# DeepMed-Lab-ECNU/BCP

Measured on AMD Instinct MI355X. Metric: training volumes/sec (LA 112x112x80 V-Net, BCP self-training step), higher is better.
Workload: dtype f32 (fp16x2 split operands); 1 GPU; LA 3D V-Net BCP self-train step, per-GPU batch 4 (2 labeled), 112x112x80 patches, SGD m0.9 wd1e-4, EMA 0.99 (BASELINE.json configs[1]); global_batch=4, parallelism=dp1

## Files before the change

bcp_amd/_lib.py:

```python
from __future__ import annotations

import ctypes as C
import os

_HERE = os.path.dirname(os.path.abspath(__file__))
LIB_PATH = os.path.join(_HERE, "csrc", "libbcp_hip.so")

ABI_VERSION = 515

P = C.c_void_p
I = C.c_int
L = C.c_longlong
F = C.c_float
U64 = C.c_ulonglong
SZ = C.c_size_t

_SIGS = {
    "bcp_version": (I, []),
    "bcp_set_option": (I, [C.c_char_p, C.c_char_p]),
    "bcp_comm_available": (I, []),
    "bcp_comm_unique_id": (I, [P]),
    "bcp_comm_init_rank": (I, [C.POINTER(P), I, I, P]),
    "bcp_comm_count": (I, [P, C.POINTER(I)]),
    "bcp_allreduce_f32": (I, [P, P, C.c_longlong, P]),
# ... 50 lines not shown
    "bcp_conv3_fwd_stats": (I, [P, P, P, P, I, I, I, I, I, I, I, P, P, I, P, P]),
    "bcp_conv3_wgrad_workspace_bytes": (SZ, [I, I, I, I, I, I, I]),
    "bcp_conv3_wgrad": (I, [P, P, P, I, I, I, I, I, I, I, I, P, P, P, P]),
    "bcp_conv3_c1_fwd": (I, [P, P, P, P, I, I, I, I, I, P]),
    "bcp_conv3_c1_stat_rows": (I, [I, I, I, I, I, I]),
    "bcp_conv3_c1_fwd_stats": (I, [P, P, P, P, I, I, I, I, I, P, I, P]),
    "bcp_conv3_c1_norm_workspace_bytes": (SZ, [I, I, I, I, I, I]),
    "bcp_conv3_c1_norm_fwd": (I, [P, P, P, I, I, I, I, I, I, P, P, P, P, F, F, I, P, F, P, F, P, P, P, P, P]),
    "bcp_conv3_c1_norm_bwd": (I, [P, P, P, P, I, I, I, I, I, I, P, I, P, F, P, F, P, P, I, P, P, P]),
    "bcp_conv3_c1_norm_bwd_wgrad_workspace_bytes": (SZ, [I, I, I, I, I, I]),
    "bcp_conv3_c1_norm_bwd_wgrad": (I, [P, P, P, P, I, I, I, I, I, I, P, I, P, F, P, F, P, P, I, P, P, I, P]),
    "bcp_conv3_c1_wgrad": (I, [P, P, P, I, I, I, I, I, I, P, P]),
    "bcp_k2_pack_weight": (I, [P, P, I, I, I, P]),
    "bcp_k2_pack_desc": (I, [P, P, I, I, I, P]),
    "bcp_k2_pack_many": (I, [P, I, P]),
    "bcp_down_fwd": (I, [P, P, P, P, I, I, I, I, I, I, P]),
    "bcp_down_dgrad": (I, [P, P, P, I, I, I, I, I, I, I, P]),
    "bcp_up_fwd": (I, [P, P, P, P, I, I, I, I, I, I, P]),
    "bcp_up_dgrad": (I, [P, P, P, I, I, I, I, I, I, I, P]),
    "bcp_k2_stat_rows": (I, [I, I, I, I, I, I, I, I]),
    "bcp_down_fwd_stats": (I, [P, P, P, P, I, I, I, I, I, I, P, I, P]),
    "bcp_up_fwd_stats": (I, [P, P, P, P, I, I, I, I, I, I, P, I, P]),
    "bcp_k2_bwdstat_rows": (I, [I, I, I, I, I, I, I, I]),
    "bcp_down_dgrad_bwdstats": (I, [P, P, P, I, I, I, I, I, I, I, P, P, I, P, I, P]),
    "bcp_up_dgrad_bwdstats": (I, [P, P, P, I, I, I, I, I, I, I, P, P, I, P, I, P]),
    "bcp_up_norm_rows": (I, [I, I, I, I, I, I, I]),
    "bcp_up_norm_workspace_bytes": (SZ, [I, I, I, I, I, I, I]),
    "bcp_up_fwd_norm": (I, [P, P, P, I, I, I, I, I, I, I, P, P, P, P, F, F, I, P, P, P, P, P, P]),
    "bcp_up_norm_bwd": (I, [P, P, P, P, I, I, I, I, I, I, I, P, I, P, P, I, P, P, P]),
    "bcp_pw_fwd": (I, [P, P, P, P, L, I, I, P]),
# ... 91 lines not shown

class Binding:

    def __init__(self, path: str):
        if not os.path.exists(path):
            raise BcpError(
                f"{path} is missing: the HIP extension has not been built.  Run "
                "`python -c 'import __graft_entry__ as g; g.build()'` (hipcc --offload-arch=gfx950). "
                "There is no CPU fallback for the product path.")
        self.path = path
        self.cdll = C.CDLL(path)
        for name, (res, args) in _SIGS.items():
            fn = getattr(self.cdll, name)
            fn.restype = res
            fn.argtypes = args
        self._status_fns = {n for n, (r, _) in _SIGS.items() if r is I and n not in ("bcp_version", "bcp_conv3_stat_rows", "bcp_comm_available", "bcp_replay_count", "bcp_norm_slabs_ok", "bcp_conv3_planes", "bcp_conv3_fwd_nslabs", "bcp_conv3_bwdstat_rows", "bcp_conv3_c1_stat_rows", "bcp_k2_stat_rows", "bcp_k2_bwdstat_rows", "bcp_conv3_last_section", "bcp_up_norm_rows")}
        self._fns = {n: (getattr(self.cdll, n), n in self._status_fns) for n in _SIGS}
        got = int(self.cdll.bcp_version())
        if got != ABI_VERSION:
            raise BcpError(f"{path}: ABI revision {got}, this binding was written against {ABI_VERSION} (include/bcp_hip.h) -- rebuild: "
                           "python -c 'import __graft_entry__ as g; g.build()'")
        self._rec = None
        self.options_epoch = 0

    def last_error(self) -> str:
        return self.cdll.bcp_last_error().decode("utf-8", "replace")

    def set_option(self, name: str, value="") -> None:
        if isinstance(value, (tuple, list)):
            value = ",".join(str(int(v)) for v in value)
        self.call("bcp_set_option", name.encode(), str(value).encode())
# ... 26 lines not shown
```

bcp_amd/csrc/api.hip:

```cpp
#include "common.h"
#include "../../include/bcp_hip.h"
#include <cstring>

namespace bcp {
static thread_local char g_err[512] = "";
void set_error(const char* fmt, ...) {
  va_list ap;
  va_start(ap, fmt);
  vsnprintf(g_err, sizeof(g_err), fmt, ap);
  va_end(ap);
}
Options& options() {
  static Options o;
  return o;
}
}

extern "C" int bcp_version(void) { return BCP_ABI_VERSION; }

extern "C" int bcp_set_option(const char* name, const char* value) {
  BCP_REQUIRE(name && value, "bcp_set_option: null argument");
  bcp::Options& o = bcp::options();
  const bcp::Options def;
  long long v[5] = {0, 0, 0, 0, 0};
  const int n = sscanf(value, "%lld,%lld,%lld,%lld,%lld", &v[0], &v[1], &v[2], &v[3], &v[4]);
  const bool reset = n <= 0;
#define BCP_OPT_INT(field) if (!strcmp(name, #field)) { o.field = reset ? def.field : (int)v[0]; return BCP_OK; }
  BCP_OPT_INT(conv3_p) BCP_OPT_INT(splitk) BCP_OPT_INT(conv3_b6_flat_sk) BCP_OPT_INT(conv3_b6_cfg2d) BCP_OPT_INT(conv3_b6_w22) BCP_OPT_INT(conv3_b6_pipe) BCP_OPT_INT(conv3_b6_cin16max) BCP_OPT_INT(res_pcu) BCP_OPT_INT(res_nt) BCP_OPT_INT(wgrad_nt)
  BCP_OPT_INT(tn_groups) BCP_OPT_INT(cc_tile) BCP_OPT_INT(pack_sections) BCP_OPT_INT(cc_select_blocks) BCP_OPT_INT(conv3_b6) BCP_OPT_INT(conv3_b6_levels) BCP_OPT_INT(conv3_b6_direct) BCP_OPT_INT(conv3_b6_flat) BCP_OPT_INT(conv3_b6_minvox) BCP_OPT_INT(wgrad_b6) BCP_OPT_INT(wgrad_b6_minvox) BCP_OPT_INT(wgrad_b6_levels) BCP_OPT_INT(wgrad_b6_slots) BCP_OPT_INT(cc_border_dedupe) BCP_OPT_INT(cc_count_tile) BCP_OPT_INT(cc_fuse_select) BCP_OPT_INT(gemm_walk) BCP_OPT_INT(gemm_pipe) BCP_OPT_INT(gemm_stat_r) BCP_OPT_INT(norm_apply_cap) BCP_OPT_INT(norm_apply_vec) BCP_OPT_INT(k2_stats) BCP_OPT_INT(k2_bwd_stats) BCP_OPT_INT(up_recompute) BCP_OPT_INT(wgrad_b6_deep) BCP_OPT_INT(wgrad_b6_deep_nt) BCP_OPT_INT(wgrad_b6_deep_slots) BCP_OPT_INT(wgrad_b6_deep_tile) BCP_OPT_INT(norm_slabs) BCP_OPT_INT(conv3_f16) BCP_OPT_INT(fuse_bwd_stats) BCP_OPT_INT(conv3_xcd) BCP_OPT_INT(mix_c1) BCP_OPT_INT(whatif) BCP_OPT_INT(c3d16_form) BCP_OPT_INT(norm_own) BCP_OPT_INT(wgrad_reduce_flat) BCP_OPT_INT(norm_fin_rows) BCP_OPT_INT(norm_fuse_fin)
#undef BCP_OPT_INT
  if (!strcmp(name, "conv3_sk_elems")) { o.conv3_sk_elems = reset ? def.conv3_sk_elems : v[0]; return BCP_OK; }
  if (!strcmp(name, "res_tile2d_vox")) { o.res_tile2d_vox = reset ? def.res_tile2d_vox : v[0]; return BCP_OK; }
  if (!strcmp(name, "conv3_cfg")) {
    BCP_REQUIRE(reset || n == 4, "bcp_set_option: conv3_cfg wants TD,TH,TW,NT");
    for (int i = 0; i < 4; ++i) o.conv3_cfg[i] = reset ? 0 : (int)v[i];
    return BCP_OK;
  }
  if (!strcmp(name, "wgrad_tile")) {
    BCP_REQUIRE(reset || n >= 3, "bcp_set_option: wgrad_tile wants TD,TH,TW[,min_voxels,max_voxels]");
    for (int i = 0; i < 5; ++i) o.wgrad_tile[i] = def.wgrad_tile[i];
    for (int i = 0; i < n && !reset; ++i) o.wgrad_tile[i] = v[i];
    return BCP_OK;
  }
  bcp::set_error("bcp_set_option: unknown option '%s'", name);
// ... 74 lines not shown
```

bcp_amd/csrc/common.h:

```cpp
#pragma once
#include <hip/hip_runtime.h>
#include <cstdarg>
#include <cstdint>
#include <cstdio>

#define BCP_OK 0
#define BCP_EINVAL (-1)
#define BCP_ELAUNCH (-2)
#define BCP_EUNSUP (-3)

typedef float f32x4 __attribute__((ext_vector_type(4)));

namespace bcp {

void set_error(const char* fmt, ...);

#define BCP_REQUIRE(cond, ...)          \
  do {                                  \
    if (!(cond)) {                      \
      ::bcp::set_error(__VA_ARGS__);    \
      return BCP_EINVAL;                \
    }                                   \
  } while (0)

// ... 46 lines not shown
  int up_recompute = 0;
  int k2_bwd_stats = 0;
  int norm_fuse_fin = 1;
  int norm_fin_rows = 128;
  int gemm_pipe = 1;
  int gemm_stat_r = 0;
  int gemm_walk = 0;
  int cc_border_dedupe = 1;
  int cc_count_tile = 0;
  int cc_fuse_select = 1;
  int norm_apply_cap = 2048;
  int norm_apply_vec = 4;
  int wgrad_reduce_flat = 1;
  int norm_own = 0;
  int c3d16_form = 1;
  int whatif = 0;
  int wgrad_b6_levels = 15;
};
Options& options();

__device__ __forceinline__ unsigned char plabel_bin_of(float x0, float x1, float thres) {
  const float m = fmaxf(x0, x1);
  const float e0 = expf(x0 - m), e1 = expf(x1 - m);
  const float p1 = e1 / (e0 + e1);
  return (p1 >= thres) ? 1 : 0;
}
__device__ __forceinline__ unsigned char plabel_argmax4_of(float x0, float x1, float x2, float x3) {
  const float m = fmaxf(fmaxf(x0, x1), fmaxf(x2, x3));
  const float e0 = expf(x0 - m), e1 = expf(x1 - m), e2 = expf(x2 - m), e3 = expf(x3 - m);
  const float s = e0 + e1 + e2 + e3;
// ... 8 lines not shown


static inline int cdiv(long long a, long long b) { return (int)((a + b - 1) / b); }
static inline bool aligned16(const void* p) { return (reinterpret_cast<uintptr_t>(p) & 15u) == 0; }

#ifndef BCP_LDS_BARRIER
#define BCP_LDS_BARRIER() asm volatile("s_waitcnt lgkmcnt(0)\n\ts_barrier" ::: "memory")
#endif

#ifndef BCP_GLDS16
typedef __attribute__((address_space(3))) void* bcp_lds_ptr_t;
#define BCP_GLDS16(gsrc, lds_wave_base) __builtin_amdgcn_global_load_lds((gsrc), (bcp_lds_ptr_t)(lds_wave_base), 16, 0, 0)
#define BCP_VM_LDS_BARRIER(N) asm volatile("s_waitcnt vmcnt(%0) lgkmcnt(0)\n\ts_barrier" ::"n"(N) : "memory")
#endif

#ifndef BCP_S_SLEEP
#define BCP_S_SLEEP(n) __builtin_amdgcn_s_sleep(n)
#endif

__device__ __forceinline__ float wave_sum(float v) {
#pragma unroll
  for (int o = 32; o > 0; o >>= 1) v += __shfl_xor(v, o);
  return v;
}
__device__ __forceinline__ double wave_sum(double v) {
#pragma unroll
  for (int o = 32; o > 0; o >>= 1) v += __shfl_xor(v, o);
  return v;
}

// ... 78 lines not shown
```

bcp_amd/csrc/gemm.hip:

```cpp
#include "common.h"
#include <cstring>
#include <cstdlib>
#include "../../include/bcp_hip.h"

namespace bcp {

enum { MAP_PLAIN = 0, MAP_PATCH = 1 };

struct RowMap {
  float* p;
  int mode;
  int L;
  int Cs;
  int D, H, W;
  __device__ __forceinline__ long long base(int m) const {
    if (mode == MAP_PLAIN) return (long long)m * L;
    const int Wc = W >> 1, Hc = H >> 1, Dc = D >> 1;
    const int wc = m % Wc, hc = (m / Wc) % Hc, dc = (m / (Wc * Hc)) % Dc, n = m / (Wc * Hc * Dc);
    return ((((long long)n * D + 2 * dc) * H + 2 * hc) * W + 2 * wc) * Cs;
  }
  __device__ __forceinline__ long long off16(int q16) const {
    if (mode == MAP_PLAIN) return q16;
    const int s = q16 / Cs, c = q16 - s * Cs;
    const int pw = s & 1, ph = (s >> 1) & 1, pd = s >> 2;
// ... 130 lines not shown
    for (int nt = 0; nt < NT; ++nt) {
      float* o = crow + C.off16(n0 + nt * 16);
      float4 v = make_float4(acc[nt][0], acc[nt][1], acc[nt][2], acc[nt][3]);
      if (bias) {
        const float4 bv = ld4(bias + (n0 + nt * 16) % bias_mod + lg * 4);
        v.x += bv.x; v.y += bv.y; v.z += bv.z; v.w += bv.w;
      }
      if (accumulate) { const float4 p = ld4(o); v.x += p.x; v.y += p.y; v.z += p.z; v.w += p.w; }
      if constexpr (STATS <= 2 || STATS == 7) st4(o, v);
      if constexpr (STATS == 3) {
        p1[nt][0] += v.x; p2[nt][0] = fmaf(v.x, v.x, p2[nt][0]);
        p1[nt][1] += v.y; p2[nt][1] = fmaf(v.y, v.y, p2[nt][1]);
        p1[nt][2] += v.z; p2[nt][2] = fmaf(v.z, v.z, p2[nt][2]);
        p1[nt][3] += v.w; p2[nt][3] = fmaf(v.w, v.w, p2[nt][3]);
      }
      if constexpr (STATS >= 4) {
        const int cb = (n0 + nt * 16) % st.C + lg * 4;
        const long long pi = (long long)(blockIdx.x / st.wpg) * st.C + cb, GC = (long long)st.G * st.C;
        const float4 mu = ld4(st.bstats + pi), rs = ld4(st.bstats + GC + pi), sc = ld4(st.bstats + 2 * GC + pi), sh = ld4(st.bstats + 3 * GC + pi);
        const float yy[4] = {v.x, v.y, v.z, v.w};
        const float m4[4] = {mu.x, mu.y, mu.z, mu.w}, r4[4] = {rs.x, rs.y, rs.z, rs.w}, s4[4] = {sc.x, sc.y, sc.z, sc.w}, h4[4] = {sh.x, sh.y, sh.z, sh.w};
        float ov[4];
        if constexpr (STATS == 4) {
          float4 rv = make_float4(0.f, 0.f, 0.f, 0.f);
          if (st.aux) rv = ld4(st.aux + (o - C.p));
          const float rr[4] = {rv.x, rv.y, rv.z, rv.w};
#pragma unroll
          for (int r = 0; r < 4; ++r) {
            const float z = (yy[r] - m4[r]) * s4[r] + h4[r];
            ov[r] = act_fwd(z, st.act);
            if (st.aux) ov[r] += rr[r];
// ... 85 lines not shown
    const int g = blockIdx.x / st.wpg, row = (blockIdx.x % st.wpg) * st.ysets + blockIdx.y / ychan;
    const int c0 = (blockIdx.y % ychan) * CT;
    if ((int)threadIdx.x < ntc * 16) {
      const int c = threadIdx.x;
      double a = 0.0, b = 0.0;
#pragma unroll
      for (int w = 0; w < 4; ++w) { a += Ss[(w * CT + c) * 2]; b += Ss[(w * CT + c) * 2 + 1]; }
      double* dst = st.partial + (((long long)g * st.nb + row) * st.C + c0 + c) * 2;
      dst[0] = a;
      dst[1] = b;
    }
    }
  }
}

template <int NT>
__global__ __launch_bounds__(256) void k_gemm_tn(RowMap A, RowMap B, float* __restrict__ partial, int M, int K, int N,
                                                 int rows_per_group) {
  constexpr int CT = NT * 16;
  constexpr int AS2 = 64 + 16;
  constexpr int BS2 = (CT % 32 == 0) ? CT + 16 : CT;
  constexpr int NB4 = (64 * (CT / 4) + 255) / 256;
  __shared__ __attribute__((aligned(16))) float As[64 * AS2];
  __shared__ __attribute__((aligned(16))) float Bs[64 * BS2];
  __shared__ long long rbase[2][2][64];
  const int lane = threadIdx.x & 63, wave = threadIdx.x >> 6;
  const int li = lane & 15, lg = lane >> 4;
  const int grp = blockIdx.x, k0 = blockIdx.y * 64, n0 = blockIdx.z * CT;
  const int r_begin = grp * rows_per_group;
  int r_end = r_begin + rows_per_group;
// ... 457 lines not shown
  if (i < C) out[i] = (accumulate ? out[i] : 0.f) + (float)accum[i];
}

static RowMap make_map(const float* p, int mode, int L, int Cs, int D, int H, int W) {
  RowMap m;
  m.p = const_cast<float*>(p);
  m.mode = mode; m.L = L; m.Cs = Cs; m.D = D; m.H = H; m.W = W;
  return m;
}

static int pick_nt(int N, long long row_blocks) {
  int nt = 4;
  while (nt > 1 && (N % (nt * 16) != 0)) nt >>= 1;
  while (nt > 1 && row_blocks * (N / (nt * 16)) < 256) nt >>= 1;
  return nt;
}

static int launch_nn(RowMap A, const float* Bp, const float* bias, RowMap C, int M, int K, int N, int bias_mod, int accumulate,
                     hipStream_t s) {
  const int rb = cdiv(M, 64);
  const int nt = pick_nt(N, rb);
  const dim3 grid(rb, N / (nt * 16));
  const GemmStats none{nullptr, 0, 0, 0, 0, 0, nullptr, nullptr, 0, 0, nullptr, nullptr, nullptr, 0};
  const int walk = options().gemm_walk;
  if (walk > 0 && (long long)rb * grid.y >= 2LL * walk) {
    int R = cdiv((long long)rb * grid.y, walk);
    if (R > 16) R = 16;
    GemmStats st = none;
    st.R = R;
    st.pipe = options().gemm_pipe;
    const dim3 g2(cdiv(rb, R), grid.y);
    if (nt == 4) hipLaunchKernelGGL((k_gemm_nn<4, 7>), g2, dim3(256), 0, s, A, Bp, bias, C, M, K, N, bias_mod, accumulate, st);
    else if (nt == 2) hipLaunchKernelGGL((k_gemm_nn<2, 7>), g2, dim3(256), 0, s, A, Bp, bias, C, M, K, N, bias_mod, accumulate, st);
    else hipLaunchKernelGGL((k_gemm_nn<1, 7>), g2, dim3(256), 0, s, A, Bp, bias, C, M, K, N, bias_mod, accumulate, st);
    return 0;
  }
  if (nt == 4) hipLaunchKernelGGL((k_gemm_nn<4>), grid, dim3(256), 0, s, A, Bp, bias, C, M, K, N, bias_mod, accumulate, none);
  else if (nt == 2) hipLaunchKernelGGL((k_gemm_nn<2>), grid, dim3(256), 0, s, A, Bp, bias, C, M, K, N, bias_mod, accumulate, none);
  else hipLaunchKernelGGL((k_gemm_nn<1>), grid, dim3(256), 0, s, A, Bp, bias, C, M, K, N, bias_mod, accumulate, none);
  return 0;
}

struct StatPlan { int nt, R, wpg, ysets, nb; };
static bool stat_plan(StatPlan& p, int M, int N, int Cout, int groups) {
  if (groups < 1 || M % groups) return false;
  const int mpg = M / groups;
  if (mpg % 64) return false;
  const int bpg = mpg / 64;
  p.nt = pick_nt(N, (long long)bpg * groups);
  const int CT = p.nt * 16;
  if (Cout % 16 || (Cout < CT && CT % Cout) || (Cout > CT && Cout % CT) || N % Cout) return false;
// ... 98 lines not shown
  BCP_REQUIRE(w && bp && desc_out && Cin > 0 && Cout > 0, "bcp_k2_pack_desc: bad argument");
  BCP_REQUIRE(Cin % 16 == 0 && Cout % 16 == 0, "bcp_k2_pack_desc: channels must be multiples of 16");
  static_assert(sizeof(GemmPackDesc) == 64, "descriptor layout is part of the ABI");
  GemmPackDesc d;
  d.w = w; d.bp = bp;
  BCP_REQUIRE(k2_pack_geometry(Cin, Cout, kind, d.K, d.N, d.ix) == 0, "bcp_k2_pack_desc: unknown kind %d", kind);
  memcpy(desc_out, &d, sizeof(d));
  return BCP_OK;
}

extern "C" int bcp_k2_pack_many(const void* descs_dev, int n, void* stream) {
  BCP_REQUIRE(descs_dev && n > 0, "bcp_k2_pack_many: bad argument");
  hipLaunchKernelGGL(k_pack_gemm_b_many, dim3(256, n), dim3(256), 0, (hipStream_t)stream, (const GemmPackDesc*)descs_dev);
  BCP_CHECK_LAUNCH("bcp_k2_pack_many");
  return BCP_OK;
}

extern "C" int bcp_down_fwd(const float* x, const float* bp, const float* bias, float* y, int N, int D, int H, int W, int Cin,
                            int Cout, void* stream) {
  BCP_REQUIRE(x && bp && y, "bcp_down_fwd: null pointer");
  BCP_REQUIRE(D % 2 == 0 && H % 2 == 0 && W % 2 == 0 && Cin % 16 == 0 && Cout % 16 == 0, "bcp_down_fwd: bad shape");
  const int M = N * (D / 2) * (H / 2) * (W / 2);
  launch_nn(make_map(x, MAP_PATCH, 8 * Cin, Cin, D, H, W), bp, bias, make_map(y, MAP_PLAIN, Cout, 0, 0, 0, 0), M, 8 * Cin, Cout,
            Cout, 0, (hipStream_t)stream);
  BCP_CHECK_LAUNCH("bcp_down_fwd");
  return BCP_OK;
}

extern "C" int bcp_k2_stat_rows(int kind, int N, int D, int H, int W, int Cin, int Cout, int groups) {
  if (N < 1 || D < 2 || H < 2 || W < 2 || (D | H | W) & 1 || Cin % 16 || Cout % 16 || Cin < 16 || Cout < 16 || groups < 1) return 0;
// ... 341 lines not shown
```

bcp_amd/csrc/replay_shapes.inc:

```
BCP_SHAPE(pifpppiiiiiipp, (void*, int, float, void*, void*, void*, int, int, int, int, int, int, void*, void*), (a[0].p, a[1].i, a[2].f, a[3].p, a[4].p, a[5].p, a[6].i, a[7].i, a[8].i, a[9].i, a[10].i, a[11].i, a[12].p, a[13].p))
BCP_SHAPE(piiiipiip, (void*, int, int, int, int, void*, int, int, void*), (a[0].p, a[1].i, a[2].i, a[3].i, a[4].i, a[5].p, a[6].i, a[7].i, a[8].p))
BCP_SHAPE(piiiippp, (void*, int, int, int, int, void*, void*, void*), (a[0].p, a[1].i, a[2].i, a[3].i, a[4].i, a[5].p, a[6].p, a[7].p))
BCP_SHAPE(piiippp, (void*, int, int, int, void*, void*, void*), (a[0].p, a[1].i, a[2].i, a[3].i, a[4].p, a[5].p, a[6].p))
BCP_SHAPE(piliippfipppppippp, (void*, int, long long, int, int, void*, void*, float, int, void*, void*, void*, void*, void*, int, void*, void*, void*), (a[0].p, a[1].i, a[2].l, a[3].i, a[4].i, a[5].p, a[6].p, a[7].f, a[8].i, a[9].p, a[10].p, a[11].p, a[12].p, a[13].p, a[14].i, a[15].p, a[16].p, a[17].p))
BCP_SHAPE(pilippppffiplpfpfppppiplpp, (void*, int, long long, int, void*, void*, void*, void*, float, float, int, void*, long long, void*, float, void*, float, void*, void*, void*, void*, int, void*, long long, void*, void*), (a[0].p, a[1].i, a[2].l, a[3].i, a[4].p, a[5].p, a[6].p, a[7].p, a[8].f, a[9].f, a[10].i, a[11].p, a[12].l, a[13].p, a[14].f, a[15].p, a[16].f, a[17].p, a[18].p, a[19].p, a[20].p, a[21].i, a[22].p, a[23].l, a[24].p, a[25].p))
BCP_SHAPE(pilippppffiplpipppippp, (void*, int, long long, int, void*, void*, void*, void*, float, float, int, void*, long long, void*, int, void*, void*, void*, int, void*, void*, void*), (a[0].p, a[1].i, a[2].l, a[3].i, a[4].p, a[5].p, a[6].p, a[7].p, a[8].f, a[9].f, a[10].i, a[11].p, a[12].l, a[13].p, a[14].i, a[15].p, a[16].p, a[17].p, a[18].i, a[19].p, a[20].p, a[21].p))
BCP_SHAPE(pilppilippppffiplpfpfpppppp, (void*, int, long long, void*, void*, int, long long, int, void*, void*, void*, void*, float, float, int, void*, long long, void*, float, void*, float, void*, void*, void*, void*, void*, void*), (a[0].p, a[1].i, a[2].l, a[3].p, a[4].p, a[5].i, a[6].l, a[7].i, a[8].p, a[9].p, a[10].p, a[11].p, a[12].f, a[13].f, a[14].i, a[15].p, a[16].l, a[17].p, a[18].f, a[19].p, a[20].f, a[21].p, a[22].p, a[23].p, a[24].p, a[25].p, a[26].p))
BCP_SHAPE(pip, (void*, int, void*), (a[0].p, a[1].i, a[2].p))
BCP_SHAPE(pipiiiippp, (void*, int, void*, int, int, int, int, void*, void*, void*), (a[0].p, a[1].i, a[2].p, a[3].i, a[4].i, a[5].i, a[6].i, a[7].p, a[8].p, a[9].p))
BCP_SHAPE(pipp, (void*, int, void*, void*), (a[0].p, a[1].i, a[2].p, a[3].p))
BCP_SHAPE(pippiiiiipip, (void*, int, void*, void*, int, int, int, int, int, void*, int, void*), (a[0].p, a[1].i, a[2].p, a[3].p, a[4].i, a[5].i, a[6].i, a[7].i, a[8].i, a[9].p, a[10].i, a[11].p))
BCP_SHAPE(plffipp, (void*, long long, float, float, int, void*, void*), (a[0].p, a[1].l, a[2].f, a[3].f, a[4].i, a[5].p, a[6].p))
BCP_SHAPE(plffiup, (void*, long long, float, float, int, unsigned long long, void*), (a[0].p, a[1].l, a[2].f, a[3].f, a[4].i, a[5].u, a[6].p))
BCP_SHAPE(plipipp, (void*, long long, int, void*, int, void*, void*), (a[0].p, a[1].l, a[2].i, a[3].p, a[4].i, a[5].p, a[6].p))
BCP_SHAPE(plippppfipipp, (void*, long long, int, void*, void*, void*, void*, float, int, void*, int, void*, void*), (a[0].p, a[1].l, a[2].i, a[3].p, a[4].p, a[5].p, a[6].p, a[7].f, a[8].i, a[9].p, a[10].i, a[11].p, a[12].p))
BCP_SHAPE(plippppfippp, (void*, long long, int, void*, void*, void*, void*, float, int, void*, void*, void*), (a[0].p, a[1].l, a[2].i, a[3].p, a[4].p, a[5].p, a[6].p, a[7].f, a[8].i, a[9].p, a[10].p, a[11].p))
BCP_SHAPE(plllppipiiiiippfpp, (void*, long long, long long, long long, void*, void*, int, void*, int, int, int, int, int, void*, void*, float, void*, void*), (a[0].p, a[1].l, a[2].l, a[3].l, a[4].p, a[5].p, a[6].i, a[7].p, a[8].i, a[9].i, a[10].i, a[11].i, a[12].i, a[13].p, a[14].p, a[15].f, a[16].p, a[17].p))
BCP_SHAPE(plllppipiiiiipppp, (void*, long long, long long, long long, void*, void*, int, void*, int, int, int, int, int, void*, void*, void*, void*), (a[0].p, a[1].l, a[2].l, a[3].l, a[4].p, a[5].p, a[6].i, a[7].p, a[8].i, a[9].i, a[10].i, a[11].i, a[12].i, a[13].p, a[14].p, a[15].p, a[16].p))
BCP_SHAPE(pp, (void*, void*), (a[0].p, a[1].p))
BCP_SHAPE(ppiiiiiiiiiiiiiiip, (void*, void*, int, int, int, int, int, int, int, int, int, int, int, int, int, int, int, void*), (a[0].p, a[1].p, a[2].i, a[3].i, a[4].i, a[5].i, a[6].i, a[7].i, a[8].i, a[9].i, a[10].i, a[11].i, a[12].i, a[13].i, a[14].i, a[15].i, a[16].i, a[17].p))
BCP_SHAPE(ppiiiiiip, (void*, void*, int, int, int, int, int, int, void*), (a[0].p, a[1].p, a[2].i, a[3].i, a[4].i, a[5].i, a[6].i, a[7].i, a[8].p))
BCP_SHAPE(ppiiiiiipiip, (void*, void*, int, int, int, int, int, int, void*, int, int, void*), (a[0].p, a[1].p, a[2].i, a[3].i, a[4].i, a[5].i, a[6].i, a[7].i, a[8].p, a[9].i, a[10].i, a[11].p))
BCP_SHAPE(ppiiiiiipp, (void*, void*, int, int, int, int, int, int, void*, void*), (a[0].p, a[1].p, a[2].i, a[3].i, a[4].i, a[5].i, a[6].i, a[7].i, a[8].p, a[9].p))
BCP_SHAPE(ppiiiiip, (void*, void*, int, int, int, int, int, void*), (a[0].p, a[1].p, a[2].i, a[3].i, a[4].i, a[5].i, a[6].i, a[7].p))
// ... 47 lines not shown
```

bcp_amd/hip_ops.py:

```python
from __future__ import annotations

import ctypes as C
import os

import torch

from . import _lib

ACT_NONE, ACT_RELU, ACT_LRELU = 0, 1, 2
LOSS_LA, LOSS_ACDC = 0, 1
PACK_DOWN_FWD, PACK_DOWN_DGRAD, PACK_UP_FWD, PACK_UP_DGRAD, PACK_PW_FWD, PACK_PW_DGRAD = range(6)
WG_DOWN, WG_UP, WG_PW = range(3)
CAST_I64_U8, CAST_F32_U8, CAST_U8_F32, CAST_U8_I64 = range(4)


AMAX_FLOATS, AMAX_STRIDE = 1024, 32
EDT_NOSITE = 1 << 30


def amax_slots(value, device):
    a = torch.zeros(AMAX_FLOATS, dtype=torch.float32, device=device)
    a[0] = value
    return a

# ... 693 lines not shown
    def k2_pack(self, w, Cin, Cout, kind):
        self._chk(w)
        bp = torch.empty(w.numel(), dtype=torch.float32, device=w.device)
        self.b.call("bcp_k2_pack_weight", _p(w), _p(bp), Cin, Cout, kind, self.stream(w))
        return bp

    def k2_pack_desc(self, w, bp, Cin, Cout, kind):
        import ctypes
        buf = ctypes.create_string_buffer(64)
        self.b.call("bcp_k2_pack_desc", _p(w), _p(bp), Cin, Cout, kind, ctypes.addressof(buf))
        return buf.raw

    def k2_pack_many(self, descs, n):
        self._chk(descs)
        self.b.call("bcp_k2_pack_many", _p(descs), int(n), self.stream(descs))

    def down_fwd(self, x, bp, bias, Cout, out=None):
        self._chk(x, bp, bias)
        N, D, H, W, Cin = x.shape
        if out is None:
            out = torch.empty((N, D // 2, H // 2, W // 2, Cout), dtype=torch.float32, device=x.device)
        self.b.call("bcp_down_fwd", _p(x), _p(bp), _p(bias), _p(out), N, D, H, W, Cin, Cout, self.stream(x))
        return self._no_amax(out)

    def k2_stat_rows(self, kind, xshape, Cout, groups):
        N, D, H, W, Cin = xshape
        fine = (D, H, W) if kind == 0 else (2 * D, 2 * H, 2 * W)
        return self._ws_bytes("bcp_k2_stat_rows", int(kind), N, fine[0], fine[1], fine[2], Cin, Cout, int(groups))

    def k2_fwd_stats(self, kind, x, bp, bias, Cout, groups):
# ... 365 lines not shown
```

include/bcp_hip.h:

```cpp
#ifndef BCP_HIP_H
#define BCP_HIP_H
#include <stddef.h>
#include <stdint.h>

#ifdef __cplusplus
extern "C" {
#endif

#define BCP_OK 0
#define BCP_EINVAL (-1)
#define BCP_ELAUNCH (-2)
#define BCP_EUNSUP (-3)

enum { BCP_ACT_NONE = 0, BCP_ACT_RELU = 1, BCP_ACT_LRELU = 2 };
enum { BCP_LOSS_LA = 0, BCP_LOSS_ACDC = 1 };
enum { BCP_CAST_I64_U8 = 0, BCP_CAST_F32_U8 = 1, BCP_CAST_U8_F32 = 2, BCP_CAST_U8_I64 = 3 };
enum { BCP_PACK_DOWN_FWD = 0, BCP_PACK_DOWN_DGRAD = 1, BCP_PACK_UP_FWD = 2, BCP_PACK_UP_DGRAD = 3, BCP_PACK_PW_FWD = 4, BCP_PACK_PW_DGRAD = 5 };
enum { BCP_WG_DOWN = 0, BCP_WG_UP = 1, BCP_WG_PW = 2 };

#define BCP_ABI_VERSION 515
int bcp_version(void);
const char* bcp_last_error(void);
int bcp_set_option(const char* name, const char* value);
int bcp_device_arch(char* buf, int n);
int bcp_event_create(void** ev);
int bcp_event_record(void* ev, void* stream);
int bcp_event_elapsed_ms(void* start, void* stop, float* ms);
int bcp_event_destroy(void* ev);

int bcp_mix_box(const float* a, const float* b, float* out, int N, int D, int H, int W, int C, const int* box6 , void* stream);

int bcp_mask_boxes(uint8_t* out, int N, int D, int H, int W, const int* boxes , int K, int complement, void* stream);
int bcp_mix_mask(const float* a, const float* b, const uint8_t* mask, float* out, int N, int D, int H, int W, long long mask_sample_stride,
                 void* stream);

// ... 109 lines not shown
int bcp_conv3_c1_norm_bwd(const float* x, const float* w, const float* bias_or_null, const float* da, int N, int D, int H, int W, int KD,
                          int groups, const float* stats, int act, const uint8_t* elem_mask, float elem_scale,
                          const unsigned long long* mask_seed_or_null, float mask_p_keep, float* dgamma, float* dbeta,
                          int accumulate, void* workspace, float* dy, void* stream);
int bcp_conv3_c1_wgrad(const float* x, const float* dy, float* dw, int N, int D, int H, int W, int KD, int accumulate, void* workspace,
                       void* stream);
size_t bcp_conv3_c1_norm_bwd_wgrad_workspace_bytes(int N, int D, int H, int W, int KD, int groups);
int bcp_conv3_c1_norm_bwd_wgrad(const float* x, const float* w, const float* bias_or_null, const float* da, int N, int D, int H, int W, int KD,
                                int groups, const float* stats, int act, const uint8_t* elem_mask, float elem_scale,
                                const unsigned long long* mask_seed_or_null, float mask_p_keep, float* dgamma, float* dbeta,
                                int accumulate, void* workspace, float* dw, int dw_accumulate, void* stream);

int bcp_k2_pack_weight(const float* w, float* bp , int Cin, int Cout, int kind, void* stream);
int bcp_k2_pack_desc(const float* w, float* bp, int Cin, int Cout, int kind, void* desc_out );
int bcp_k2_pack_many(const void* descs_dev, int n, void* stream);
int bcp_down_fwd(const float* x, const float* bp, const float* bias, float* y, int N, int D, int H, int W, int Cin, int Cout, void* stream);
int bcp_down_dgrad(const float* dy, const float* bp, float* dx, int N, int D, int H, int W, int Cin, int Cout, int accumulate, void* stream);
int bcp_up_fwd(const float* x, const float* bp, const float* bias, float* y, int N, int D, int H, int W, int Cin, int Cout, void* stream);
int bcp_k2_stat_rows(int kind, int N, int D, int H, int W, int Cin, int Cout, int groups);
int bcp_down_fwd_stats(const float* x, const float* bp, const float* bias, float* y, int N, int D, int H, int W, int Cin, int Cout, double* stat_partial, int groups, void* stream);
int bcp_up_fwd_stats(const float* x, const float* bp, const float* bias, float* y, int N, int D, int H, int W, int Cin, int Cout, double* stat_partial, int groups, void* stream);
int bcp_k2_bwdstat_rows(int kind, int N, int D, int H, int W, int Cin, int Cout, int groups);
int bcp_down_dgrad_bwdstats(const float* dy, const float* bp, float* dx, int N, int D, int H, int W, int Cin, int Cout, int accumulate, const float* y_prev, const float* stats_prev, int act, double* stat_partial, int groups, void* stream);
int bcp_up_dgrad_bwdstats(const float* dy, const float* bp, float* dx, int N, int D, int H, int W, int Cin, int Cout, int accumulate, const float* y_prev, const float* stats_prev, int act, double* stat_partial, int groups, void* stream);
int bcp_up_norm_rows(int N, int D, int H, int W, int Cin, int Cout, int groups);
size_t bcp_up_norm_workspace_bytes(int N, int D, int H, int W, int Cin, int Cout, int groups);
int bcp_up_fwd_norm(const float* x, const float* bp, const float* bias, int N, int D, int H, int W, int Cin, int Cout, int groups, const float* gamma, const float* beta, float* running_mean, float* running_var, float momentum, float eps, int act, const float* residual_or_null, float* stats, void* workspace, float* out, float* amax_out_or_null, void* stream);
int bcp_up_norm_bwd(const float* x, const float* bp, const float* bias, const float* da, int N, int D, int H, int W, int Cin, int Cout, int groups, const float* stats, int act, float* dgamma, float* dbeta, int accumulate, void* workspace, float* dy, void* stream);
int bcp_up_dgrad(const float* dy, const float* bp, float* dx, int N, int D, int H, int W, int Cin, int Cout, int accumulate, void* stream);
int bcp_pw_fwd(const float* x, const float* bp, const float* bias_or_null, float* y, long long rows, int Cin, int Cout, void* stream);
// ... 83 lines not shown
```

Measured before the change: 814.1 volumes/s.

## Add multi-stage async LDS-pipelined NN GEMM kernel for large-K down/up convs

Adds a new NN GEMM kernel that prefetches four K-stages of A and B into LDS through direct global-to-LDS loads, with graded vmcnt barriers and explicit ds_read_b128 register staging ahead of the MFMA chain. It is enabled by default (gemm_kpipe=1) for non-stats, non-walk NN launches with K of at least 256, and aims to hide global memory latency in the k2 down/up/pointwise GEMMs. The kernel uses far more LDS, which may limit occupancy to two workgroups per CU. A path-query entry point and an option are also added.

```diff
diff --git a/bcp_amd/_lib.py b/bcp_amd/_lib.py
--- a/bcp_amd/_lib.py
+++ b/bcp_amd/_lib.py
@@ -6,7 +6,7 @@
 _HERE = os.path.dirname(os.path.abspath(__file__))
 LIB_PATH = os.path.join(_HERE, "csrc", "libbcp_hip.so")
 
-ABI_VERSION = 515
+ABI_VERSION = 516
 
 P = C.c_void_p
 I = C.c_int
@@ -88,6 +88,7 @@
     "bcp_k2_pack_weight": (I, [P, P, I, I, I, P]),
     "bcp_k2_pack_desc": (I, [P, P, I, I, I, P]),
     "bcp_k2_pack_many": (I, [P, I, P]),
+    "bcp_gemm_nn_path": (I, [L, I, I]),
     "bcp_down_fwd": (I, [P, P, P, P, I, I, I, I, I, I, P]),
     "bcp_down_dgrad": (I, [P, P, P, I, I, I, I, I, I, I, P]),
     "bcp_up_fwd": (I, [P, P, P, P, I, I, I, I, I, I, P]),
@@ -209,7 +210,7 @@
             fn = getattr(self.cdll, name)
             fn.restype = res
             fn.argtypes = args
-        self._status_fns = {n for n, (r, _) in _SIGS.items() if r is I and n not in ("bcp_version", "bcp_conv3_stat_rows", "bcp_comm_available", "bcp_replay_count", "bcp_norm_slabs_ok", "bcp_conv3_planes", "bcp_conv3_fwd_nslabs", "bcp_conv3_bwdstat_rows", "bcp_conv3_c1_stat_rows", "bcp_k2_stat_rows", "bcp_k2_bwdstat_rows", "bcp_conv3_last_section", "bcp_up_norm_rows")}
+        self._status_fns = {n for n, (r, _) in _SIGS.items() if r is I and n not in ("bcp_version", "bcp_conv3_stat_rows", "bcp_comm_available", "bcp_replay_count", "bcp_norm_slabs_ok", "bcp_conv3_planes", "bcp_conv3_fwd_nslabs", "bcp_conv3_bwdstat_rows", "bcp_conv3_c1_stat_rows", "bcp_k2_stat_rows", "bcp_k2_bwdstat_rows", "bcp_conv3_last_section", "bcp_up_norm_rows", "bcp_gemm_nn_path")}
         self._fns = {n: (getattr(self.cdll, n), n in self._status_fns) for n in _SIGS}
         got = int(self.cdll.bcp_version())
         if got != ABI_VERSION:
diff --git a/bcp_amd/csrc/api.hip b/bcp_amd/csrc/api.hip
--- a/bcp_amd/csrc/api.hip
+++ b/bcp_amd/csrc/api.hip
@@ -27,7 +27,7 @@
   const bool reset = n <= 0;
 #define BCP_OPT_INT(field) if (!strcmp(name, #field)) { o.field = reset ? def.field : (int)v[0]; return BCP_OK; }
   BCP_OPT_INT(conv3_p) BCP_OPT_INT(splitk) BCP_OPT_INT(conv3_b6_flat_sk) BCP_OPT_INT(conv3_b6_cfg2d) BCP_OPT_INT(conv3_b6_w22) BCP_OPT_INT(conv3_b6_pipe) BCP_OPT_INT(conv3_b6_cin16max) BCP_OPT_INT(res_pcu) BCP_OPT_INT(res_nt) BCP_OPT_INT(wgrad_nt)
-  BCP_OPT_INT(tn_groups) BCP_OPT_INT(cc_tile) BCP_OPT_INT(pack_sections) BCP_OPT_INT(cc_select_blocks) BCP_OPT_INT(conv3_b6) BCP_OPT_INT(conv3_b6_levels) BCP_OPT_INT(conv3_b6_direct) BCP_OPT_INT(conv3_b6_flat) BCP_OPT_INT(conv3_b6_minvox) BCP_OPT_INT(wgrad_b6) BCP_OPT_INT(wgrad_b6_minvox) BCP_OPT_INT(wgrad_b6_levels) BCP_OPT_INT(wgrad_b6_slots) BCP_OPT_INT(cc_border_dedupe) BCP_OPT_INT(cc_count_tile) BCP_OPT_INT(cc_fuse_select) BCP_OPT_INT(gemm_walk) BCP_OPT_INT(gemm_pipe) BCP_OPT_INT(gemm_stat_r) BCP_OPT_INT(norm_apply_cap) BCP_OPT_INT(norm_apply_vec) BCP_OPT_INT(k2_stats) BCP_OPT_INT(k2_bwd_stats) BCP_OPT_INT(up_recompute) BCP_OPT_INT(wgrad_b6_deep) BCP_OPT_INT(wgrad_b6_deep_nt) BCP_OPT_INT(wgrad_b6_deep_slots) BCP_OPT_INT(wgrad_b6_deep_tile) BCP_OPT_INT(norm_slabs) BCP_OPT_INT(conv3_f16) BCP_OPT_INT(fuse_bwd_stats) BCP_OPT_INT(conv3_xcd) BCP_OPT_INT(mix_c1) BCP_OPT_INT(whatif) BCP_OPT_INT(c3d16_form) BCP_OPT_INT(norm_own) BCP_OPT_INT(wgrad_reduce_flat) BCP_OPT_INT(norm_fin_rows) BCP_OPT_INT(norm_fuse_fin)
+  BCP_OPT_INT(tn_groups) BCP_OPT_INT(cc_tile) BCP_OPT_INT(pack_sections) BCP_OPT_INT(cc_select_blocks) BCP_OPT_INT(conv3_b6) BCP_OPT_INT(conv3_b6_levels) BCP_OPT_INT(conv3_b6_direct) BCP_OPT_INT(conv3_b6_flat) BCP_OPT_INT(conv3_b6_minvox) BCP_OPT_INT(wgrad_b6) BCP_OPT_INT(wgrad_b6_minvox) BCP_OPT_INT(wgrad_b6_levels) BCP_OPT_INT(wgrad_b6_slots) BCP_OPT_INT(cc_border_dedupe) BCP_OPT_INT(cc_count_tile) BCP_OPT_INT(cc_fuse_select) BCP_OPT_INT(gemm_walk) BCP_OPT_INT(gemm_pipe) BCP_OPT_INT(gemm_stat_r) BCP_OPT_INT(norm_apply_cap) BCP_OPT_INT(norm_apply_vec) BCP_OPT_INT(k2_stats) BCP_OPT_INT(k2_bwd_stats) BCP_OPT_INT(up_recompute) BCP_OPT_INT(wgrad_b6_deep) BCP_OPT_INT(wgrad_b6_deep_nt) BCP_OPT_INT(wgrad_b6_deep_slots) BCP_OPT_INT(wgrad_b6_deep_tile) BCP_OPT_INT(norm_slabs) BCP_OPT_INT(conv3_f16) BCP_OPT_INT(fuse_bwd_stats) BCP_OPT_INT(conv3_xcd) BCP_OPT_INT(mix_c1) BCP_OPT_INT(whatif) BCP_OPT_INT(c3d16_form) BCP_OPT_INT(gemm_kpipe) BCP_OPT_INT(norm_own) BCP_OPT_INT(wgrad_reduce_flat) BCP_OPT_INT(norm_fin_rows) BCP_OPT_INT(norm_fuse_fin)
 #undef BCP_OPT_INT
   if (!strcmp(name, "conv3_sk_elems")) { o.conv3_sk_elems = reset ? def.conv3_sk_elems : v[0]; return BCP_OK; }
   if (!strcmp(name, "res_tile2d_vox")) { o.res_tile2d_vox = reset ? def.res_tile2d_vox : v[0]; return BCP_OK; }
diff --git a/bcp_amd/csrc/common.h b/bcp_amd/csrc/common.h
--- a/bcp_amd/csrc/common.h
+++ b/bcp_amd/csrc/common.h
@@ -84,6 +84,7 @@
   int wgrad_reduce_flat = 1;
   int norm_own = 0;
   int c3d16_form = 1;
+  int gemm_kpipe = 1;
   int whatif = 0;
   int wgrad_b6_levels = 15;
 };
@@ -122,6 +123,15 @@
 #define BCP_VM_LDS_BARRIER(N) asm volatile("s_waitcnt vmcnt(%0) lgkmcnt(0)\n\ts_barrier" ::"n"(N) : "memory")
 #endif
 
+#ifndef BCP_LDS_READ16
+#define BCP_LDS_READ16(dst, p, byte_off) \
+  asm volatile("ds_read_b128 %0, %1 offset:%2" : "=v"(dst) : "v"((unsigned)(uintptr_t)(bcp_lds_ptr_t)(p)), "n"(byte_off) : "memory")
+#define BCP_LDS_LANDED4(a, b, c, d) asm volatile("s_waitcnt lgkmcnt(0)" : "+v"(a), "+v"(b), "+v"(c), "+v"(d))
+#define BCP_LDS_LANDED6(a, b, c, d, e, f) asm volatile("s_waitcnt lgkmcnt(0)" : "+v"(a), "+v"(b), "+v"(c), "+v"(d), "+v"(e), "+v"(f))
+#define BCP_LDS_LANDED10(a, b, c, d, e, f, g, h, i, j) \
+  asm volatile("s_waitcnt lgkmcnt(0)" : "+v"(a), "+v"(b), "+v"(c), "+v"(d), "+v"(e), "+v"(f), "+v"(g), "+v"(h), "+v"(i), "+v"(j))
+#endif
+
 #ifndef BCP_S_SLEEP
 #define BCP_S_SLEEP(n) __builtin_amdgcn_s_sleep(n)
 #endif
diff --git a/bcp_amd/csrc/gemm.hip b/bcp_amd/csrc/gemm.hip
--- a/bcp_amd/csrc/gemm.hip
+++ b/bcp_amd/csrc/gemm.hip
@@ -168,7 +168,7 @@
         p1[nt][2] += v.z; p2[nt][2] = fmaf(v.z, v.z, p2[nt][2]);
         p1[nt][3] += v.w; p2[nt][3] = fmaf(v.w, v.w, p2[nt][3]);
       }
-      if constexpr (STATS >= 4) {
+      if constexpr (STATS >= 4 && STATS <= 6) {
         const int cb = (n0 + nt * 16) % st.C + lg * 4;
         const long long pi = (long long)(blockIdx.x / st.wpg) * st.C + cb, GC = (long long)st.G * st.C;
         const float4 mu = ld4(st.bstats + pi), rs = ld4(st.bstats + GC + pi), sc = ld4(st.bstats + 2 * GC + pi), sh = ld4(st.bstats + 3 * GC + pi);
@@ -284,6 +284,117 @@
   }
 }
 
+template <int P, int A>
+__device__ __forceinline__ void kp_stage_barrier(const int ahead) {
+  if constexpr (A == 0) BCP_VM_LDS_BARRIER(0);
+  else {
+    if (ahead >= A) BCP_VM_LDS_BARRIER(A * P);
+    else kp_stage_barrier<P, A - 1>(ahead);
+  }
+}
+
+static constexpr int KPS = 4;
+
+template <int NT>
+__global__ __launch_bounds__(256) void k_gemm_nn_kp(RowMap A, const float* __restrict__ Bp, const float* __restrict__ bias,
+                                                    RowMap C, int M, int K, int N, int bias_mod, int accumulate) {
+  constexpr int CT = NT * 16;
+  constexpr int NB = NT >= 2 ? NT / 2 : 1;
+  constexpr int P = 2 + NB;
+  constexpr int ASZ = 64 * KC, BSZ = 8 * CT * 4;
+  HIP_DYNAMIC_SHARED(float4, smem4)
+  float* const As = reinterpret_cast<float*>(smem4);
+  float* const Bs = As + KPS * ASZ;
+  const int lane = threadIdx.x & 63, wave = threadIdx.x >> 6;
+  const int li = lane & 15, lg = lane >> 4;
+  const int n0 = blockIdx.y * CT, m0 = blockIdx.x * 64;
+
+  const int srow = threadIdx.x >> 2, spart = threadIdx.x & 3;
+  const float* arow = A.p + ((m0 + srow) < M ? A.base(m0 + srow) : 0) + spart * 4;
+  static_assert(NB <= 2, "k_gemm_nn_kp: at most 64-column slabs");
+  long long boff[2];
+#pragma unroll
+  for (int u = 0; u < NB; ++u) {
+    const int q = (threadIdx.x + u * 256) % (8 * CT);
+    boff[u] = ((long long)(q / CT) * N + n0 + q % CT) * 4;
+  }
+  const int wave_u = __builtin_amdgcn_readfirstlane(wave);
+  float* const a_dst = As + wave_u * 256;
+  float* const b_dst = Bs + (NT == 1 ? (wave_u & 1) : wave_u) * 256;
+  const int seg_len = A.mode == MAP_PLAIN ? A.L : A.Cs;
+  int seg_c = 0, seg_s = 0, islot = 0;
+  long long seg_off = 0;
+  const float* bnext = Bp;
+  auto issue = [&]() __attribute__((always_inline)) {
+#pragma unroll
+    for (int h = 0; h < 2; ++h) {
+      BCP_GLDS16(arow + seg_off + seg_c, a_dst + islot * ASZ + h * 1024);
+      seg_c += 16;
+      if (seg_c == seg_len) {
+        seg_c = 0;
+        ++seg_s;
+        seg_off = ((((long long)(seg_s >> 2) * A.H + ((seg_s >> 1) & 1)) * A.W + (seg_s & 1))) * A.Cs;
+      }
+    }
+#pragma unroll
+    for (int u = 0; u < NB; ++u) BCP_GLDS16(bnext + boff[u], b_dst + islot * BSZ + u * 1024);
+    bnext += (long long)KC * N;
+    islot = (islot + 1) & (KPS - 1);
+  };
+
+  f32x4 acc[NT];
+#pragma unroll
+  for (int nt = 0; nt < NT; ++nt) acc[nt] = (f32x4){0.f, 0.f, 0.f, 0.f};
+
+  const int nst = K / KC;
+#pragma unroll
+  for (int s = 0; s < KPS - 1; ++s)
+    if (s < nst) issue();
+#pragma unroll 1
+  for (int i = 0; i < nst; ++i) {
+    static_assert((KPS - 2) * P < 64, "vmcnt is a 6-bit count");
+    kp_stage_barrier<P, KPS - 2>(nst - 1 - i);
+    if (i + KPS - 1 < nst) issue();
+    const float* as = As + (i & (KPS - 1)) * ASZ + (wave * 16 + li) * 16 + lg * 4;
+    const float* bs = Bs + (i & (KPS - 1)) * BSZ + (lg * CT + li) * 4;
+    f32x4 a[2], b[2][4];
+#pragma unroll
+    for (int kq = 0; kq < KC / 16; ++kq) {
+      BCP_LDS_READ16(a[kq], as, kq * 4096);
+#pragma unroll
+      for (int nt = 0; nt < NT; ++nt) BCP_LDS_READ16(b[kq][nt], bs, (kq * 4 * CT + nt * 16) * 16);
+    }
+    if constexpr (NT == 1) BCP_LDS_LANDED4(a[0], a[1], b[0][0], b[1][0]);
+    else if constexpr (NT == 2) BCP_LDS_LANDED6(a[0], a[1], b[0][0], b[0][1], b[1][0], b[1][1]);
+    else BCP_LDS_LANDED10(a[0], a[1], b[0][0], b[0][1], b[0][2], b[0][3], b[1][0], b[1][1], b[1][2], b[1][3]);
+#pragma unroll
+    for (int kq = 0; kq < KC / 16; ++kq) {
+#pragma unroll
+      for (int nt = 0; nt < NT; ++nt) {
+        acc[nt] = __builtin_amdgcn_mfma_f32_16x16x4f32(b[kq][nt].x, a[kq].x, acc[nt], 0, 0, 0);
+        acc[nt] = __builtin_amdgcn_mfma_f32_16x16x4f32(b[kq][nt].y, a[kq].y, acc[nt], 0, 0, 0);
+        acc[nt] = __builtin_amdgcn_mfma_f32_16x16x4f32(b[kq][nt].z, a[kq].z, acc[nt], 0, 0, 0);
+        acc[nt] = __builtin_amdgcn_mfma_f32_16x16x4f32(b[kq][nt].w, a[kq].w, acc[nt], 0, 0, 0);
+      }
+    }
+  }
+  const int mr = m0 + wave * 16 + li;
+  if (mr < M) {
+    float* crow = C.p + C.base(mr) + lg * 4;
+#pragma unroll
+    for (int nt = 0; nt < NT; ++nt) {
+      float* o = crow + C.off16(n0 + nt * 16);
+      float4 v = make_float4(acc[nt][0], acc[nt][1], acc[nt][2], acc[nt][3]);
+      if (bias) {
+        const float4 bv = ld4(bias + (n0 + nt * 16) % bias_mod + lg * 4);
+        v.x += bv.x; v.y += bv.y; v.z += bv.z; v.w += bv.w;
+      }
+      if (accumulate) { const float4 p = ld4(o); v.x += p.x; v.y += p.y; v.z += p.z; v.w += p.w; }
+      st4(o, v);
+    }
+  }
+}
+
 template <int NT>
 __global__ __launch_bounds__(256) void k_gemm_tn(RowMap A, RowMap B, float* __restrict__ partial, int M, int K, int N,
                                                  int rows_per_group) {
@@ -771,6 +882,21 @@
   while (nt > 1 && (N % (nt * 16) != 0)) nt >>= 1;
   while (nt > 1 && row_blocks * (N / (nt * 16)) < 256) nt >>= 1;
   return nt;
+}
+
+static constexpr int kKpipeMinK = 256;
+template <int NT>
+static void launch_kp(dim3 grid, hipStream_t s, RowMap A, const float* Bp, const float* bias, RowMap C, int M, int K, int N, int bias_mod,
+                      int accumulate) {
+  constexpr size_t lds = (size_t)KPS * (64 * KC + 8 * NT * 16 * 4) * sizeof(float);
+  static_assert(2 * lds <= 160 * 1024, "two workgroups per CU");
+  auto kfn = k_gemm_nn_kp<NT>;
+  if (lds > 48 * 1024) hipFuncSetAttribute(reinterpret_cast<const void*>(kfn), hipFuncAttributeMaxDynamicSharedMemorySize, (int)lds);
+  hipLaunchKernelGGL(kfn, grid, dim3(256), lds, s, A, Bp, bias, C, M, K, N, bias_mod, accumulate);
+}
+static bool kpipe_eligible(int K) {
+  const int v = options().gemm_kpipe;
+  return v > 0 && K % KC == 0 && K >= (v > 1 ? v : kKpipeMinK);
 }
 
 static int launch_nn(RowMap A, const float* Bp, const float* bias, RowMap C, int M, int K, int N, int bias_mod, int accumulate,
@@ -792,6 +918,12 @@
     else hipLaunchKernelGGL((k_gemm_nn<1, 7>), g2, dim3(256), 0, s, A, Bp, bias, C, M, K, N, bias_mod, accumulate, st);
     return 0;
   }
+  if (kpipe_eligible(K)) {
+    if (nt == 4) launch_kp<4>(grid, s, A, Bp, bias, C, M, K, N, bias_mod, accumulate);
+    else if (nt == 2) launch_kp<2>(grid, s, A, Bp, bias, C, M, K, N, bias_mod, accumulate);
+    else launch_kp<1>(grid, s, A, Bp, bias, C, M, K, N, bias_mod, accumulate);
+    return 0;
+  }
   if (nt == 4) hipLaunchKernelGGL((k_gemm_nn<4>), grid, dim3(256), 0, s, A, Bp, bias, C, M, K, N, bias_mod, accumulate, none);
   else if (nt == 2) hipLaunchKernelGGL((k_gemm_nn<2>), grid, dim3(256), 0, s, A, Bp, bias, C, M, K, N, bias_mod, accumulate, none);
   else hipLaunchKernelGGL((k_gemm_nn<1>), grid, dim3(256), 0, s, A, Bp, bias, C, M, K, N, bias_mod, accumulate, none);
@@ -920,6 +1052,14 @@
   hipLaunchKernelGGL(k_pack_gemm_b_many, dim3(256, n), dim3(256), 0, (hipStream_t)stream, (const GemmPackDesc*)descs_dev);
   BCP_CHECK_LAUNCH("bcp_k2_pack_many");
   return BCP_OK;
+}
+
+extern "C" int bcp_gemm_nn_path(long long M, int K, int N) {
+  if (M < 1 || K < 1 || N < 16 || N % 16) return 0;
+  const int rb = cdiv(M, 64), nt = pick_nt(N, rb);
+  const int walk = options().gemm_walk;
+  if (walk > 0 && (long long)rb * (N / (nt * 16)) >= 2LL * walk) return 0;
+  return kpipe_eligible(K) ? nt : 0;
 }
 
 extern "C" int bcp_down_fwd(const float* x, const float* bp, const float* bias, float* y, int N, int D, int H, int W, int Cin,
diff --git a/bcp_amd/csrc/replay_shapes.inc b/bcp_amd/csrc/replay_shapes.inc
--- a/bcp_amd/csrc/replay_shapes.inc
+++ b/bcp_amd/csrc/replay_shapes.inc
@@ -1,3 +1,4 @@
+BCP_SHAPE(lii, (long long, int, int), (a[0].l, a[1].i, a[2].i))
 BCP_SHAPE(pifpppiiiiiipp, (void*, int, float, void*, void*, void*, int, int, int, int, int, int, void*, void*), (a[0].p, a[1].i, a[2].f, a[3].p, a[4].p, a[5].p, a[6].i, a[7].i, a[8].i, a[9].i, a[10].i, a[11].i, a[12].p, a[13].p))
 BCP_SHAPE(piiiipiip, (void*, int, int, int, int, void*, int, int, void*), (a[0].p, a[1].i, a[2].i, a[3].i, a[4].i, a[5].p, a[6].i, a[7].i, a[8].p))
 BCP_SHAPE(piiiippp, (void*, int, int, int, int, void*, void*, void*), (a[0].p, a[1].i, a[2].i, a[3].i, a[4].i, a[5].p, a[6].p, a[7].p))
diff --git a/bcp_amd/hip_ops.py b/bcp_amd/hip_ops.py
--- a/bcp_amd/hip_ops.py
+++ b/bcp_amd/hip_ops.py
@@ -731,6 +731,9 @@
     def k2_pack_many(self, descs, n):
         self._chk(descs)
         self.b.call("bcp_k2_pack_many", _p(descs), int(n), self.stream(descs))
+
+    def gemm_nn_path(self, M, K, N):
+        return self._ws_bytes("bcp_gemm_nn_path", int(M), int(K), int(N))
 
     def down_fwd(self, x, bp, bias, Cout, out=None):
         self._chk(x, bp, bias)
diff --git a/include/bcp_hip.h b/include/bcp_hip.h
--- a/include/bcp_hip.h
+++ b/include/bcp_hip.h
@@ -18,7 +18,7 @@
 enum { BCP_PACK_DOWN_FWD = 0, BCP_PACK_DOWN_DGRAD = 1, BCP_PACK_UP_FWD = 2, BCP_PACK_UP_DGRAD = 3, BCP_PACK_PW_FWD = 4, BCP_PACK_PW_DGRAD = 5 };
 enum { BCP_WG_DOWN = 0, BCP_WG_UP = 1, BCP_WG_PW = 2 };
 
-#define BCP_ABI_VERSION 515
+#define BCP_ABI_VERSION 516
 int bcp_version(void);
 const char* bcp_last_error(void);
 int bcp_set_option(const char* name, const char* value);
@@ -158,6 +158,7 @@
 int bcp_k2_pack_weight(const float* w, float* bp , int Cin, int Cout, int kind, void* stream);
 int bcp_k2_pack_desc(const float* w, float* bp, int Cin, int Cout, int kind, void* desc_out );
 int bcp_k2_pack_many(const void* descs_dev, int n, void* stream);
+int bcp_gemm_nn_path(long long M, int K, int N);
 int bcp_down_fwd(const float* x, const float* bp, const float* bias, float* y, int N, int D, int H, int W, int Cin, int Cout, void* stream);
 int bcp_down_dgrad(const float* dy, const float* bp, float* dx, int N, int D, int H, int W, int Cin, int Cout, int accumulate, void* stream);
 int bcp_up_fwd(const float* x, const float* bp, const float* bias, float* y, int N, int D, int H, int W, int Cin, int Cout, void* stream);
```

Result: no change. 821.3 volumes/s (median of 6 runs) (+0.9%).
